# daovietanh190499/3D_Reconstruction

Measured on AMD Instinct MI355X. Metric: image-pairs matched/sec, higher is better.
Workload: dtype f32 descriptors: int8 MFMA certified filter + f64 re-score; 1 GPU; C3/C4 all-pairs BF-L2 + ratio 0.75: 257 imgs x 4096 kpts x 256-d, exact f32-input semantics (oracle.match.bf_match_exact, bit for bit); pairs=32896, api=dist.match_all_pairs_sharded(exact=True), match_mode=exact-float, parallelism=pairs/1

## Files before the change

### 3d_reconstruction_amd/csrc/fp6_sched.h

```cpp
#pragma once

namespace sfmhip {

template <int KK, int NS>
struct Fp6Sched {
    static constexpr int MPT = KK * NS;
    static constexpr int F = (KK - 1) * NS + 5;
    static constexpr int kBudget = KK == 1 ? 3 : 2;
    static_assert(F + 1 < MPT, "a spilled maximum reads its chain before the next tile rewrites it");
    static constexpr int chain(int g, int which) { return (g - F - which + MPT) % MPT; }
    static constexpr bool back(int g, int which) { return g - F - which < 0; }
    static constexpr int load(int g) { return (chain(g, 0) < NS) + (chain(g, 1) < NS); }
    static constexpr int before(int g, int which) {
        const int f = F + which, wrap = f + NS - MPT;
        return (g < wrap ? g : wrap) + (g > f ? g - f : 0);
    }
    static constexpr int merge(int h, int j) {
        const int g = h % MPT;
        const int k = (h / MPT) * (kBudget * MPT - 2 * NS) + kBudget * g - before(g, 0) - before(g, 1);
        return (j < kBudget - load(g) && k + j < 4 * NS) ? k + j : -1;
    }
    static constexpr int merge_chain(int k) { return 2 * (k / 8) + ((0xCA >> (k % 8)) & 1); }
    static constexpr int merge_step(int k) { return (0x3232'1100 >> (4 * (k % 8))) & 15; }
    static constexpr int kOwedFirst = MPT - F, kOwedSecond = MPT - F - 1;
    static constexpr bool merge_ready() {
        for (int c = 0; c < NS; ++c) {
            int h = 0;
            while (true) {
                bool found = false;
                for (int j = 0; j < kBudget; ++j) found |= merge(h, j) == 8 * (c / 2) + c % 2;
                if (found) break;
                ++h;
            }
            if (h < F + 1 + c - MPT) return false;
        }
        return true;
    }
};

__device__ __forceinline__ void fp6_merge_step(int step, float m, int rid, bool& up, float& w1, float& w2, int& wr) {
    const float a = w1, b = w2;
    const int r = wr;
    const bool u = up;
    if (step == 0) up = m > a;
    else if (step == 1) w2 = __builtin_amdgcn_fmed3f(a, b, m);
    else if (step == 2) wr = u ? rid : r;
    else w1 = u ? m : a;
}

}
```

### 3d_reconstruction_amd/csrc/match_dev.h

```cpp
#pragma once

#include "common.h"
#include <climits>

namespace sfmhip {

typedef int i32x2 __attribute__((ext_vector_type(2)));
typedef int i32x4 __attribute__((ext_vector_type(4)));
typedef int i32x8 __attribute__((ext_vector_type(8)));
typedef float f32x4 __attribute__((ext_vector_type(4)));

constexpr int kJB = 128;

template <int D>
__device__ __forceinline__ int swz_off(int r, int c) {
    constexpr int CPR = D / 16;
    constexpr int RPB = 256 / D;
    return r * D + ((c ^ ((r / RPB) % CPR)) << 4);
}

__device__ __forceinline__ int max3i(int a, int b, int c) {
    int r;
    asm("v_max3_i32 %0, %1, %2, %3" : "=v"(r) : "v"(a), "v"(b), "v"(c));
    return r;
}
__device__ __forceinline__ int med3i(int a, int b, int c) {
    int r;
    asm("v_med3_i32 %0, %1, %2, %3" : "=v"(r) : "v"(a), "v"(b), "v"(c));
    return r;
}

template <int D, int WAVES>
struct Stager {
    static constexpr int CPR = D / 16;
    static constexpr int RPB = 256 / D;
    static constexpr int TILE = kJB * D;
    static constexpr int NI = TILE / 1024;
    static constexpr int PER_WAVE = NI / WAVES;
    static constexpr int LDT = TILE / 16 / (64 * WAVES);
    static_assert(NI % WAVES == 0 && LDT >= 1, "block / workgroup mismatch");

    __device__ static void dma(const int8_t* src, const int32_t* ksrc, int8_t* dst, int32_t* kdst, int wave,
                               int lane) {
#pragma unroll
        for (int u = 0; u < PER_WAVE; ++u) {
            const int ins = wave * PER_WAVE + u;
            const int rows_per_ins = 1024 / D;
            const int r0 = ins * rows_per_ins;
            const int r = r0 + lane / CPR;
            const int c = (lane % CPR) ^ ((r / RPB) % CPR);
            __builtin_amdgcn_global_load_lds(
                (__attribute__((address_space(1))) void*)(src + (size_t)r * D + c * 16),
                (__attribute__((address_space(3))) void*)(dst + r0 * D), 16, 0, 0);
        }
        if (wave == WAVES - 1) {
#pragma unroll
            for (int u = 0; u < 2; ++u)
                __builtin_amdgcn_global_load_lds(
                    (__attribute__((address_space(1))) void*)(ksrc + u * 64 + lane),
                    (__attribute__((address_space(3))) void*)(kdst + u * 64), 4, 0, 0);
        }
    }
};

template <int MF> struct Mfma;
template <> struct Mfma<16> {
    using acc_t = i32x4;
    static constexpr int NREG = 4, KB = 64;
    __device__ static acc_t run(i32x4 a, i32x4 b, acc_t c) {
        return __builtin_amdgcn_mfma_i32_16x16x64_i8(a, b, c, 0, 0, 0);
    }
    __device__ static int row(int q, int grp) { return 4 * grp + q; }
};

struct CertArgs {
    const double* erow;
    const double* eimg;
    double inv_s;
    int force;
};
constexpr int kUndecidedBase = -3;
constexpr int kValueOnlyTiles = 4;
__device__ __forceinline__ int sqrt8_ceil(int d2) {
    const long long t = 64LL * d2;
    int u = (int)ceil(sqrt((double)t));
    while (u > 0 && (long long)(u - 1) * (u - 1) >= t) --u;
    while ((long long)u * u < t) ++u;
    return u;
}
template <typename OutT>
__device__ __forceinline__ int undecided_mark(int d2) {
    if constexpr (sizeof(OutT) == 2) return kUndecidedBase - sqrt8_ceil(d2);
    else return kUndecidedBase - d2;
}
template <typename OutT>
__device__ __forceinline__ double mark_sqrt_d2(int mark) {
    if constexpr (sizeof(OutT) == 2) return (double)(kUndecidedBase - mark) * 0.125;
    else return sqrt((double)(kUndecidedBase - mark));
}

__device__ __forceinline__ int certify(int d1lo, int d1hi, int d2lo, int d2hi, double E, double inv_s, double rn2,
                                       double rd2) {
    const double up = 1.0 + 0x1p-50, dn = 1.0 - 0x1p-50;
    const double s1l = sqrt((double)d1lo) * inv_s, s1h = sqrt((double)d1hi) * inv_s;
    const double s2l = sqrt((double)d2lo) * inv_s, s2h = sqrt((double)d2hi) * inv_s;
    const double a1 = fmax(s1l * dn - E * up, 0.0), b1 = (s1h + E) * up;
    const double a2 = fmax(s2l * dn - E * up, 0.0), b2 = (s2h + E) * up;
    const double wl = 1.0 - 1e-12, wh = 1.0 + 1e-12;
    const double lo1 = a1 * a1 * wl, hi1 = b1 * b1 * wh, lo2 = a2 * a2 * wl, hi2 = b2 * b2 * wh;
    if (rd2 * lo1 >= rn2 * hi2) return 0;
    if (hi1 < lo2 && rd2 * hi1 < rn2 * lo2) return 1;
    return -1;
}

template <int D, int MF, int NS, int VG, typename OutT>
__device__ __forceinline__ void value_only_tail(const int (&w1)[NS], const int (&w2)[NS], const int (&wr)[NS],
                                                const int8_t* __restrict__ desc, const int8_t* __restrict__ bdesc,
                                                const int32_t* __restrict__ bkeys, const int32_t* __restrict__ norms,
                                                int a, int b, int m_pad, int na_rows, int ibase, int grp, int lr,
                                                int lane, long long rn2, long long rd2, OutT* __restrict__ out_m,
                                                const CertArgs& ca) {
    constexpr int NG = 64 / MF;
    int v1 = INT_MIN, v2 = INT_MIN, loc = 0;
#pragma unroll
    for (int s = 0; s < NS; ++s) {
        int a1 = w1[s], a2 = w2[s], al = wr[s] * NG + grp;
#pragma unroll
        for (int off = MF; off < 64; off <<= 1) {
            const int o1 = __shfl_xor(a1, off), o2 = __shfl_xor(a2, off), ol = __shfl_xor(al, off);
            const bool mine = a1 > o1 || (a1 == o1 && al < ol);
            a2 = max3i(min(a1, o1), a2, o2);
            al = mine ? al : ol;
            a1 = max(a1, o1);
        }
        if (s == grp) { v1 = a1; v2 = a2; loc = al; }
    }
    const int i = ibase + grp * MF + lr;
    int res = -1, na = 0, du1 = 0, hidx = -1;
    double E = 0.0;
    bool survivor = false;
    if (i < na_rows) {
        na = norms[(size_t)a * m_pad + i];
        du1 = na - 2 * v1;
        const int du2ub = na - 2 * v2;
        E = ca.erow[(size_t)a * m_pad + i] + ca.eimg[b];
        if (ca.force)
            res = undecided_mark<OutT>(min(du2ub, D * 255 * 255));
        else
            survivor = certify(max(du1 - 1, 0), du1, max(du1 - 1, 0), du2ub, E, ca.inv_s, (double)rn2,
                               (double)rd2) != 0;
    }
    constexpr int NC = 4 * VG;
    constexpr int LPC = (64 / NC) < (D / 16) ? (64 / NC) : (D / 16);
    constexpr int BPL = D / LPC;
    const int c = min(lane / LPC, NC - 1), part = lane % LPC;
    unsigned long long bal = __ballot(survivor);
    while (bal) {
        const int l = __builtin_ctzll(bal);
        bal &= bal - 1;
        const int ri = __shfl(i, l), rv = __shfl(v1, l), rl = __shfl(loc, l);
        const int j0 = (rl / NG) * VG * MF + 4 * (rl % NG);
        const int j = j0 + (c >> 2) * MF + (c & 3);
        const int8_t* pa = desc + ((size_t)a * m_pad + ri) * D + part * BPL;
        const int8_t* pb = bdesc + (size_t)j * D + part * BPL;
        int dot = 0;
#pragma unroll
        for (int w = 0; w < BPL / 16; ++w) {
            const i32x4 x = *reinterpret_cast<const i32x4*>(pa + 16 * w);
            const i32x4 y = *reinterpret_cast<const i32x4*>(pb + 16 * w);
#pragma unroll
            for (int e = 0; e < 4; ++e) dot = __builtin_amdgcn_sdot4(x[e], y[e], dot, false);
        }
#pragma unroll
        for (int off = 1; off < LPC; off <<= 1) dot += __shfl_xor(dot, off);
        const int u = dot + bkeys[j];
        const bool hit = lane < NC * LPC && part == 0 && u == rv;
        const unsigned long long hb = __ballot(hit);
        int x = u == rv ? INT_MIN : u;
#pragma unroll
        for (int off = LPC; off < 64; off <<= 1) x = max(x, __shfl_xor(x, off));
        if (lane == l) {
            const bool one = __popcll(hb) == 1;
            v2 = max(v2, one ? x : rv);
            if (one) {
                const int hc = __builtin_ctzll(hb) / LPC;
                hidx = j0 + (hc >> 2) * MF + (hc & 3);
            }
        }
    }
    if (survivor) {
        const int du2 = na - 2 * v2;
        const int v = certify(max(du1 - 1, 0), du1, max(du2 - 1, 0), du2, E, ca.inv_s, (double)rn2, (double)rd2);
        res = v == 0 ? -1 : (v > 0 && hidx >= 0) ? hidx : undecided_mark<OutT>(du2);
    }
    if (i < m_pad) out_m[i] = (OutT)res;
}

constexpr int kMatchRows = 256;
constexpr int kMatchFp6Rows = 512;

struct FilterLaunch {
    const int8_t* desc;
    const int32_t* norms;
    const int32_t* keys;
    const int32_t* n_kpts;
    int m_pad, d;
    const int32_t* pairs;
    int n_iblk, nwg;
    long long rn2, rd2;
    CertArgs ca;
    hipStream_t stream;
    int32_t *dist1, *dist2;
    const uint8_t* dense;
    const float* hf;
};
template <typename OutT> int launch_match_cert(const FilterLaunch& f, OutT* matches0);
template <typename OutT> int launch_match_fp6(const FilterLaunch& f, OutT* matches0);
struct ResolveLaunch;
template <typename OutT> int launch_resolve(const ResolveLaunch& r, OutT* matches0);
void launch_key_values(const int32_t* keys, int64_t n, int32_t* h, float* hf, hipStream_t stream);

template <typename OutT>
inline int check_match_call(const char* entry, bool exact, int n_img, int P, int m_pad, int mode, int ratio_num,
                            int ratio_den, bool pointers, int rows_per_wg, int* n_iblk, int* nwg) {
    *n_iblk = *nwg = 0;
    SFMHIP_REQUIRE(n_img > 0 && P >= 0, "%s: bad counts", entry);
    SFMHIP_REQUIRE(m_pad > 0 && m_pad % kJB == 0, "%s: m_pad must be a positive multiple of 128", entry);
    if (exact) SFMHIP_REQUIRE(mode == 0 || mode == 1, "%s: mode must be 0 or 1", entry);
    SFMHIP_REQUIRE(ratio_num > 0 && ratio_den > 0 && ratio_num <= 65535 && ratio_den <= 65535,
                   "%s: ratio must be a positive fraction", entry);
    if constexpr (sizeof(OutT) == 2)
        SFMHIP_REQUIRE(m_pad <= 32767, "%s_i16: m_pad must be <= 32767 for an int16 graph", entry);
    if (P == 0) return SFMHIP_OK;
    SFMHIP_REQUIRE(pointers, "%s: null pointer", entry);
    *n_iblk = ceil_div(m_pad, rows_per_wg);
    const int64_t nwg64 = (int64_t)P * *n_iblk;
    SFMHIP_REQUIRE(nwg64 < INT_MAX, "%s: too many pairs for one launch", entry);
    *nwg = (int)nwg64;
    return SFMHIP_OK;
}

}
```

### 3d_reconstruction_amd/csrc/match_fp6.hip

```cpp
#include "match_dev.h"
#include "fp6_sched.h"

namespace sfmhip {

__device__ __forceinline__ int fp6_grid_index(float y, int* g) {
    const float t = fminf(fabsf(y), 60.f);
    int n, m;
    if (t < 16.f) { m = (int)__builtin_rintf(t); n = m; }
    else if (t < 32.f) { const int r = (int)__builtin_rintf(0.5f * t); m = 2 * r; n = r + 8; }
    else { const int r = (int)__builtin_rintf(0.25f * t); m = 4 * r; n = r + 16; }
    const bool neg = y < 0.f && m > 0;
    *g = neg ? -m : m;
    return n | (neg ? 32 : 0);
}
__global__ void quantize_fp6_kernel(const float* __restrict__ in, int64_t n_chunks, int d, int m_pad,
                                    const int32_t* __restrict__ nk, int8_t* __restrict__ g,
                                    uint8_t* __restrict__ code) {
    for (int64_t c = (int64_t)blockIdx.x * blockDim.x + threadIdx.x; c < n_chunks;
         c += (int64_t)gridDim.x * blockDim.x) {
        const int64_t e0 = c * 32, row = e0 / d;
        const int img = (int)(row / m_pad), r = (int)(row % m_pad);
        const bool valid = r < nk[img];
        unsigned gw[8], cw[8];
#pragma unroll
        for (int w = 0; w < 8; ++w) gw[w] = cw[w] = 0u;
        if (valid) {
#pragma unroll
            for (int q = 0; q < 8; ++q) {
                const float4 x = *reinterpret_cast<const float4*>(in + e0 + 4 * q);
                const float v[4] = {x.x, x.y, x.z, x.w};
                unsigned pk = 0u;
#pragma unroll
                for (int t = 0; t < 4; ++t) {
                    int gv;
                    const int cd = fp6_grid_index(127.f * v[t], &gv);
                    gw[q] |= (unsigned)(gv & 0xff) << (8 * t);
                    pk |= (unsigned)cd << (6 * t);
                }
#pragma unroll
                for (int t = 0; t < 3; ++t) {
                    const int byte = 3 * q + t;
                    cw[byte >> 2] |= ((pk >> (8 * t)) & 0xffu) << (8 * (byte & 3));
                }
            }
        }
        uint4* go = reinterpret_cast<uint4*>(g + e0);
        uint4* co = reinterpret_cast<uint4*>(code + e0);
        go[0] = make_uint4(gw[0], gw[1], gw[2], gw[3]);
        go[1] = make_uint4(gw[4], gw[5], gw[6], gw[7]);
        co[0] = make_uint4(cw[0], cw[1], cw[2], cw[3]);
        co[1] = make_uint4(cw[4], cw[5], cw[6], cw[7]);
    }
}


__global__ void pack_fp6_kernel(const uint8_t* __restrict__ code, int64_t n_chunks, int d,
                                uint8_t* __restrict__ dense) {
    const int spr = d / 32;
    for (int64_t c = (int64_t)blockIdx.x * blockDim.x + threadIdx.x; c < n_chunks;
         c += (int64_t)gridDim.x * blockDim.x) {
        const int64_t row = c / spr;
        const int s = (int)(c % spr);
        const uint4 lo = *reinterpret_cast<const uint4*>(code + c * 32);
        const uint2 hi = *reinterpret_cast<const uint2*>(code + c * 32 + 16);
        uint8_t* rp = dense + row * (3 * d / 4);
        *reinterpret_cast<uint4*>(rp + 16 * s) = lo;
        *reinterpret_cast<uint2*>(rp + d / 2 + 8 * s) = hi;
    }
}

template <int D, int WAVES>
struct DenseStager {
    static constexpr int ROW = 3 * D / 4, LB = D / 2, HB = D / 4;
    static constexpr int LO = kJB * LB, TILE = kJB * ROW;
    static constexpr int CPR = LB / 16, RPB = 256 / LB;
    static constexpr int UPR = HB / 16, RPH = 256 / HB;
    static constexpr int NLO = LO / 1024 / WAVES, NHI = (TILE - LO) / 1024 / WAVES;
    static_assert(NLO * WAVES * 1024 == LO && NHI * WAVES * 1024 == TILE - LO && NLO >= 1 && NHI >= 1,
                  "block / workgroup mismatch");
    static_assert(RPB * CPR == 16 && RPH * UPR == 16, "a 16-row tile covers every bank once");

    __device__ static int lo_sw(int r) { return ((((r & 15) + 4) >> 3) & 1) ^ ((r / RPB) % CPR); }
    __device__ static int hi_sw(int r) { return (r / RPH) % UPR; }
    __device__ static int lo_off(int r, int s) { return r * LB + ((s ^ lo_sw(r)) << 4); }
    __device__ static int hi_off(int r, int s) { return LO + r * HB + ((((s >> 1) ^ hi_sw(r)) << 4) | ((s & 1) << 3)); }

    struct Lanes {
        unsigned lo[NLO], hi[NHI], key;
    };
    __device__ static Lanes lanes(int wave, int lane) {
        Lanes l;
#pragma unroll
        for (int u = 0; u < NLO; ++u) {
            const int r = (wave * NLO + u) * (1024 / LB) + lane / CPR;
            l.lo[u] = (unsigned)(r * ROW + (((lane % CPR) ^ lo_sw(r)) << 4));
        }
#pragma unroll
        for (int u = 0; u < NHI; ++u) {
            const int r = (wave * NHI + u) * (1024 / HB) + lane / UPR;
            l.hi[u] = (unsigned)(r * ROW + LB + (((lane % UPR) ^ hi_sw(r)) << 4));
        }
        l.key = (unsigned)(lane * 4);
        return l;
    }

    __device__ static void dma(const uint8_t* src, const int32_t* ksrc, int8_t* dst, int32_t* kdst, int wave,
                               const Lanes& l) {
#pragma unroll
        for (int u = 0; u < NLO; ++u) {
            unsigned o = l.lo[u];
            asm volatile("" : "+v"(o));
            __builtin_amdgcn_global_load_lds((__attribute__((address_space(1))) void*)(src + o),
                                             (__attribute__((address_space(3))) void*)(dst + (wave * NLO + u) * 1024),
                                             16, 0, 0);
        }
#pragma unroll
        for (int u = 0; u < NHI; ++u) {
            unsigned o = l.hi[u];
            asm volatile("" : "+v"(o));
            __builtin_amdgcn_global_load_lds(
                (__attribute__((address_space(1))) void*)(src + o),
                (__attribute__((address_space(3))) void*)(dst + LO + (wave * NHI + u) * 1024), 16, 0, 0);
        }
        if (wave == WAVES - 1) {
#pragma unroll
            for (int u = 0; u < 2; ++u)
                __builtin_amdgcn_global_load_lds(
                    (__attribute__((address_space(1))) void*)(reinterpret_cast<const uint8_t*>(ksrc + u * 64) + l.key),
                    (__attribute__((address_space(3))) void*)(kdst + u * 64), 4, 0, 0);
        }
    }
};

__device__ __forceinline__ i32x2 lds_read_b64(const int8_t* p) {
    return *(const volatile __attribute__((address_space(3))) i32x2*)p;
}

struct Fp6Operand {
    i32x4 lo;
    i32x2 hi;
    __device__ i32x8 tuple() const { return i32x8{lo[0], lo[1], lo[2], lo[3], hi[0], hi[1], 0, 0}; }
};

constexpr int kFp6Tiles = 8;
constexpr int kFp6Waves = 4;

template <int D, typename OutT>
__global__ __launch_bounds__(64 * kFp6Waves, 2) void match_fp6_kernel(
    const uint8_t* __restrict__ dense, const int8_t* __restrict__ g, const int32_t* __restrict__ norms,
    const int32_t* __restrict__ h, const float* __restrict__ hf, const int32_t* __restrict__ nk, int m_pad,
    const int32_t* __restrict__ pairs, int n_iblk, int nwg, long long rn2, long long rd2,
    OutT* __restrict__ m0, CertArgs ca) {
    constexpr int MF = 16, NS = kFp6Tiles, WAVES = kFp6Waves, VG = kValueOnlyTiles;
    static_assert(D % 128 == 0, "one MFMA takes 128 elements of k");
    static_assert(NS % 4 == 0, "value_only_tail takes four query tiles at a time");
    using S = DenseStager<D, WAVES>;
    constexpr int KK = D / 128;
    using SC = Fp6Sched<KK, NS>;
    static_assert(kJB / MF == 2 * VG, "two ranges per block: the range maxima alternate between two sets");
    static_assert(SC::merge(VG * SC::MPT, 0) == -1, "a range's gaps hold the previous range's merge");
    static_assert(SC::merge_ready(), "a chain's merge starts behind its last maximum");
    constexpr int TILE = S::TILE;
    constexpr int NT = 64 * WAVES;
    constexpr int IW = MF * NS, IB = IW * WAVES;
    constexpr int JT = kJB / MF;
    constexpr int kScale = 0;
    constexpr float kLow = -262144.f;

    __shared__ __attribute__((aligned(16))) int8_t lds[2 * TILE + 2 * kJB * 4];

    const int wg = xcd_remap(blockIdx.x, nwg);
    const int pair = wg / n_iblk, ib = wg % n_iblk;
    const int a = pairs[2 * pair], b = pairs[2 * pair + 1];
    const int na_rows = nk[a], nb_rows = nk[b];
    const int tid = threadIdx.x, lane = tid & 63;
    const int wave = __builtin_amdgcn_readfirstlane(tid >> 6);
    const int grp = lane / MF, lr = lane % MF;
    const int ibase = ib * IB + wave * IW;
    OutT* out_m = m0 + (size_t)pair * m_pad;

    if (ib * IB >= na_rows || nb_rows < 2) {
        const int iend = min(ib * IB + IB, m_pad);
        for (int i = ib * IB + tid; i < iend; i += NT) out_m[i] = -1;
        return;
    }

    const uint8_t* bdense = dense + (size_t)b * m_pad * S::ROW;
    const int32_t* bhf = reinterpret_cast<const int32_t*>(hf) + (size_t)b * m_pad;
    const int nblk = (nb_rows + kJB - 1) / kJB;
    int32_t* kbase = reinterpret_cast<int32_t*>(lds + 2 * TILE);

    const typename S::Lanes dl = S::lanes(wave, lane);
    S::dma(bdense, bhf, lds, kbase, wave, dl);

    Fp6Operand bq[NS][KK];
#pragma unroll
    for (int s = 0; s < NS; ++s) {
        const int i = min(ibase + s * MF + lr, m_pad - 1);
        const uint8_t* rp = dense + ((size_t)a * m_pad + i) * S::ROW;
#pragma unroll
        for (int kk = 0; kk < KK; ++kk) {
            bq[s][kk].lo = *reinterpret_cast<const i32x4*>(rp + 16 * (kk * 4 + grp));
            bq[s][kk].hi = *reinterpret_cast<const i32x2*>(rp + S::LB + 8 * (kk * 4 + grp));
        }
    }
    int lo_b[KK], hi_b[KK];
#pragma unroll
    for (int kk = 0; kk < KK; ++kk) {
        lo_b[kk] = S::lo_off(lr, kk * 4 + grp);
        hi_b[kk] = S::hi_off(lr, kk * 4 + grp);
    }

    float w1[NS], w2[NS];
    int wr[NS];
    f32x4 acc[NS];
    float half[NS], rm[2][NS];
    bool up[NS];
    int rid_owed = 0;
#pragma unroll
    for (int s = 0; s < NS; ++s) {
        w1[s] = kLow; w2[s] = kLow; wr[s] = 0;
        acc[s] = f32x4{kLow, kLow, kLow, kLow};
        half[s] = rm[0][s] = rm[1][s] = kLow;
        up[s] = false;
    }
    auto merge_step = [&](int c, int step, float m, int rid) {
        fp6_merge_step(step, m, rid, up[c], w1[c], w2[c], wr[c]);
    };

    __syncthreads();

    const uint8_t* bsrc = bdense;
    const int32_t* ksrc = bhf;
    for (int blk = 0; blk < nblk; ++blk) {
        const int cur = blk & 1;
        bsrc += TILE;
        ksrc += kJB;
        if (blk + 1 < nblk)
            S::dma(bsrc, ksrc, lds + (cur ^ 1) * TILE, kbase + (cur ^ 1) * kJB, wave, dl);
        const int8_t* tl = lds + cur * TILE;
        const float* kl = reinterpret_cast<const float*>(kbase + cur * kJB);
        Fp6Operand av;
        av.lo = *reinterpret_cast<const i32x4*>(tl + lo_b[0]);
        av.hi = lds_read_b64(tl + hi_b[0]);
        f32x4 hv = *reinterpret_cast<const f32x4*>(kl + 4 * grp);
#pragma unroll
        for (int jt = 0; jt < JT; ++jt) {
            const int R = jt / VG, tt = jt % VG;
            f32x4 hv_n = hv;
#pragma unroll
            for (int kk = 0; kk < KK; ++kk) {
                Fp6Operand av_n = av;
                __builtin_amdgcn_sched_barrier(0);
#pragma unroll
                for (int s = 0; s < NS; ++s) {
                    acc[s] = __builtin_amdgcn_mfma_scale_f32_16x16x128_f8f6f4(av.tuple(), bq[s][kk].tuple(),
                                                                              kk == 0 ? hv : acc[s], 2, 2, 0, kScale, 0,
                                                                              kScale);
                    __builtin_amdgcn_sched_barrier(0);
                    if (s == 0) {
                        if (kk + 1 < KK) {
                            av_n.lo = *reinterpret_cast<const i32x4*>(tl + lo_b[kk + 1] + jt * MF * S::LB);
                            av_n.hi = lds_read_b64(tl + hi_b[kk + 1] + jt * MF * S::HB);
                        } else if (jt + 1 < JT) {
                            av_n.lo = *reinterpret_cast<const i32x4*>(tl + lo_b[0] + (jt + 1) * MF * S::LB);
                            av_n.hi = lds_read_b64(tl + hi_b[0] + (jt + 1) * MF * S::HB);
                            hv_n = *reinterpret_cast<const f32x4*>(kl + (jt + 1) * MF + 4 * grp);
                        }
                        __builtin_amdgcn_sched_barrier(0);
                    }
                    const int gp = kk * NS + s;
                    if (const int c = SC::chain(gp, 0); c < NS) {
                        const int of = tt - SC::back(gp, 0);
                        const float from = of < 0 ? rm[R ^ 1][c] : of == 0 ? kLow : rm[R][c];
                        half[c] = __builtin_fmaxf(__builtin_fmaxf(from, acc[c][0]), acc[c][1]);
                    }
                    if (const int c = SC::chain(gp, 1); c < NS)
                        rm[tt == 0 && SC::back(gp, 1) ? R ^ 1 : R][c] =
                            __builtin_fmaxf(__builtin_fmaxf(half[c], acc[c][2]), acc[c][3]);
#pragma unroll
                    for (int j = 0; j < SC::kBudget; ++j)
                        if (const int k = SC::merge(tt * SC::MPT + gp, j); k >= 0) {
                            __builtin_amdgcn_sched_barrier(0);
                            merge_step(SC::merge_chain(k), SC::merge_step(k), rm[R ^ 1][SC::merge_chain(k)], rid_owed);
                        }
                    __builtin_amdgcn_sched_barrier(0);
                }
                av = av_n;
            }
            hv = hv_n;
            if (tt == VG - 1) rid_owed = blk * (JT / VG) + R;
        }
        __syncthreads();
    }
#pragma unroll
    for (int s = SC::kOwedFirst; s < NS; ++s)
        half[s] = __builtin_fmaxf(__builtin_fmaxf(rm[1][s], acc[s][0]), acc[s][1]);
#pragma unroll
    for (int s = SC::kOwedSecond; s < NS; ++s)
        rm[1][s] = __builtin_fmaxf(__builtin_fmaxf(half[s], acc[s][2]), acc[s][3]);
#pragma unroll
    for (int s = 0; s < NS; ++s)
#pragma unroll
        for (int step = 0; step < 4; ++step) merge_step(s, step, rm[1][s], rid_owed);

#pragma unroll
    for (int q = 0; q < NS / 4; ++q) {
        int v1[4], v2[4], vr[4];
#pragma unroll
        for (int s = 0; s < 4; ++s) {
            v1[s] = (int)(64.f * w1[4 * q + s]);
            v2[s] = (int)(64.f * w2[4 * q + s]);
            vr[s] = wr[4 * q + s];
        }
        value_only_tail<D, MF, 4, VG, OutT>(v1, v2, vr, g, g + (size_t)b * m_pad * D, h + (size_t)b * m_pad, norms, a, b,
                                            m_pad, na_rows, ibase + q * 4 * MF, grp, lr, lane, rn2, rd2, out_m, ca);
    }
}

template <typename OutT>
int launch_match_fp6(const FilterLaunch& f, OutT* matches0) {
    static_assert(kMatchFp6Rows == 16 * kFp6Tiles * kFp6Waves, "query rows per workgroup");
    auto launch = [&](auto kern) {
        hipLaunchKernelGGL(kern, dim3(f.nwg), dim3(64 * kFp6Waves), 0, f.stream, f.dense, f.desc, f.norms, f.keys, f.hf,
                           f.n_kpts, f.m_pad, f.pairs, f.n_iblk, f.nwg, f.rn2, f.rd2, matches0, f.ca);
    };
    switch (f.d) {
        case 128: launch(match_fp6_kernel<128, OutT>); break;
        case 256: launch(match_fp6_kernel<256, OutT>); break;
        default: return SFMHIP_E_UNSUPPORTED;
    }
    return check_launch("match_kernel<cert>");
}
template int launch_match_fp6<int32_t>(const FilterLaunch&, int32_t*);
template int launch_match_fp6<int16_t>(const FilterLaunch&, int16_t*);

}

using namespace sfmhip;

extern "C" int sfmhip_desc_quantize_fp6(const float* in, int n_img, int m_pad, int d, const int32_t* n_kpts,
                                        int8_t* g, uint8_t* code, void* stream) {
    SFMHIP_REQUIRE(in && g && code && n_kpts, "sfmhip_desc_quantize_fp6: null pointer");
    SFMHIP_REQUIRE(n_img > 0 && m_pad > 0 && d > 0 && d % 32 == 0, "sfmhip_desc_quantize_fp6: bad shape");
    const int64_t n_chunks = (int64_t)n_img * m_pad * d / 32;
    const int grid = (int)std::min<int64_t>((n_chunks + 255) / 256, 4096);
    hipLaunchKernelGGL(quantize_fp6_kernel, dim3(grid), dim3(256), 0, as_stream(stream), in, n_chunks, d, m_pad,
                       n_kpts, g, code);
    return check_launch("quantize_fp6_kernel");
}

extern "C" int sfmhip_desc_pack_fp6(const uint8_t* code, int n_img, int m_pad, int d, uint8_t* dense, void* stream) {
    SFMHIP_REQUIRE(code && dense, "sfmhip_desc_pack_fp6: null pointer");
    SFMHIP_REQUIRE(n_img > 0 && m_pad > 0 && d > 0 && d % 64 == 0, "sfmhip_desc_pack_fp6: bad shape");
    const int64_t n_chunks = (int64_t)n_img * m_pad * d / 32;
    const int grid = (int)std::min<int64_t>((n_chunks + 255) / 256, 4096);
    hipLaunchKernelGGL(pack_fp6_kernel, dim3(grid), dim3(256), 0, as_stream(stream), code, n_chunks, d, dense);
    return check_launch("pack_fp6_kernel");
}
```

Baseline: 665,100 pairs/s.

## Make fp6 value-range width a per-D template parameter spanning blocks

The range width VG (column tiles per tracked maximum) becomes a template parameter chosen per descriptor size: four tiles for 256-d (unchanged from the former constant) and sixteen for 128-d, where a range now spans two blocks. The block loop is restructured into phase-specialised unrolled bodies so range sets alternate correctly across blocks, and the tail's re-scan is bounded by the last valid column. Wider ranges mean fewer merge steps in the main loop but more candidates to re-score per survivor in the tail. For the 256-d workload the default path keeps the same range size, so mainly the code structure changes.

```diff
diff --git a/3d_reconstruction_amd/csrc/fp6_sched.h b/3d_reconstruction_amd/csrc/fp6_sched.h
--- a/3d_reconstruction_amd/csrc/fp6_sched.h
+++ b/3d_reconstruction_amd/csrc/fp6_sched.h
@@ -36,6 +36,34 @@
         }
         return true;
     }
+    static constexpr bool merge_once(int tiles) {
+        int next = 0;
+        for (int h = 0; h < tiles * MPT; ++h) {
+            int n = load(h % MPT);
+            for (int j = 0; j < kBudget; ++j)
+                if (const int k = merge(h, j); k >= 0) {
+                    if (k != next) return false;
+                    ++next;
+                    ++n;
+                }
+            if (n > kBudget) return false;
+        }
+        return next == 4 * NS;
+    }
+};
+
+template <int VG, int JT>
+struct Fp6Range {
+    static_assert(VG >= 1 && (VG & (VG - 1)) == 0 && JT >= 1 && (JT & (JT - 1)) == 0, "powers of two");
+    static constexpr int PER = 2 * VG > JT ? 2 * VG / JT : 1;
+    static constexpr int set(int ph, int jt) { return ((ph * JT + jt) / VG) & 1; }
+    static constexpr int tile(int ph, int jt) { return (ph * JT + jt) % VG; }
+    static constexpr bool valid() {
+        if ((PER * JT) % (2 * VG) != 0 || set(PER - 1, JT - 1) != 1 || tile(PER - 1, JT - 1) != VG - 1) return false;
+        for (int ph = 0; ph < PER; ++ph)
+            if (tile(ph, JT - 1) == 0) return false;
+        return true;
+    }
 };
 
 __device__ __forceinline__ void fp6_merge_step(int step, float m, int rid, bool& up, float& w1, float& w2, int& wr) {
diff --git a/3d_reconstruction_amd/csrc/match_dev.h b/3d_reconstruction_amd/csrc/match_dev.h
--- a/3d_reconstruction_amd/csrc/match_dev.h
+++ b/3d_reconstruction_amd/csrc/match_dev.h
@@ -119,7 +119,7 @@
                                                 const int32_t* __restrict__ bkeys, const int32_t* __restrict__ norms,
                                                 int a, int b, int m_pad, int na_rows, int ibase, int grp, int lr,
                                                 int lane, long long rn2, long long rd2, OutT* __restrict__ out_m,
-                                                const CertArgs& ca) {
+                                                const CertArgs& ca, int j_end = INT_MAX) {
     constexpr int NG = 64 / MF;
     int v1 = INT_MIN, v2 = INT_MIN, loc = 0;
 #pragma unroll
@@ -160,7 +160,12 @@
         bal &= bal - 1;
         const int ri = __shfl(i, l), rv = __shfl(v1, l), rl = __shfl(loc, l);
         const int j0 = (rl / NG) * VG * MF + 4 * (rl % NG);
-        const int j = j0 + (c >> 2) * MF + (c & 3);
+        int j = j0 + (c >> 2) * MF + (c & 3);
+        bool seen = true;
+        if constexpr (VG * MF > kJB) {
+            seen = j < j_end;
+            j = seen ? j : j0;
+        }
         const int8_t* pa = desc + ((size_t)a * m_pad + ri) * D + part * BPL;
         const int8_t* pb = bdesc + (size_t)j * D + part * BPL;
         int dot = 0;
@@ -173,7 +178,7 @@
         }
 #pragma unroll
         for (int off = 1; off < LPC; off <<= 1) dot += __shfl_xor(dot, off);
-        const int u = dot + bkeys[j];
+        const int u = seen ? dot + bkeys[j] : INT_MIN;
         const bool hit = lane < NC * LPC && part == 0 && u == rv;
         const unsigned long long hb = __ballot(hit);
         int x = u == rv ? INT_MIN : u;
diff --git a/3d_reconstruction_amd/csrc/match_fp6.hip b/3d_reconstruction_amd/csrc/match_fp6.hip
--- a/3d_reconstruction_amd/csrc/match_fp6.hip
+++ b/3d_reconstruction_amd/csrc/match_fp6.hip
@@ -144,21 +144,46 @@
 
 constexpr int kFp6Tiles = 8;
 constexpr int kFp6Waves = 4;
-
-template <int D, typename OutT>
+#ifndef SFMHIP_FP6_RANGE_256
+#define SFMHIP_FP6_RANGE_256 4
+#endif
+#ifndef SFMHIP_FP6_RANGE_128
+#define SFMHIP_FP6_RANGE_128 16
+#endif
+template <int D>
+constexpr int kFp6RangeTiles = D == 256 ? SFMHIP_FP6_RANGE_256 : SFMHIP_FP6_RANGE_128;
+
+template <typename T>
+__device__ __forceinline__ void fp6_hold(T& x) {
+    asm volatile("" : "+v"(x));
+}
+
+template <typename T>
+__device__ __forceinline__ void fp6_hold_uniform(T& x) {
+    asm volatile("" : "+s"(x));
+}
+
+template <int K>
+struct Fp6Phase {
+    static constexpr int value = K;
+};
+
+template <int D, typename OutT, int VG = kFp6RangeTiles<D>>
 __global__ __launch_bounds__(64 * kFp6Waves, 2) void match_fp6_kernel(
     const uint8_t* __restrict__ dense, const int8_t* __restrict__ g, const int32_t* __restrict__ norms,
     const int32_t* __restrict__ h, const float* __restrict__ hf, const int32_t* __restrict__ nk, int m_pad,
     const int32_t* __restrict__ pairs, int n_iblk, int nwg, long long rn2, long long rd2,
     OutT* __restrict__ m0, CertArgs ca) {
-    constexpr int MF = 16, NS = kFp6Tiles, WAVES = kFp6Waves, VG = kValueOnlyTiles;
+    constexpr int MF = 16, NS = kFp6Tiles, WAVES = kFp6Waves;
     static_assert(D % 128 == 0, "one MFMA takes 128 elements of k");
     static_assert(NS % 4 == 0, "value_only_tail takes four query tiles at a time");
     using S = DenseStager<D, WAVES>;
     constexpr int KK = D / 128;
     using SC = Fp6Sched<KK, NS>;
-    static_assert(kJB / MF == 2 * VG, "two ranges per block: the range maxima alternate between two sets");
-    static_assert(SC::merge(VG * SC::MPT, 0) == -1, "a range's gaps hold the previous range's merge");
+    using RG = Fp6Range<VG, kJB / MF>;
+    static_assert(VG == 4 || VG == 8 || VG == 16, "ranges of half a block, one block or two blocks");
+    static_assert(RG::valid(), "the range maxima alternate between two sets by the parity of the range");
+    static_assert(SC::merge_once(VG < kJB / MF ? VG : kJB / MF), "a range's first gaps hold the previous range's merge, once");
     static_assert(SC::merge_ready(), "a chain's merge starts behind its last maximum");
     constexpr int TILE = S::TILE;
     constexpr int NT = 64 * WAVES;
@@ -230,23 +255,15 @@
 
     __syncthreads();
 
-    const uint8_t* bsrc = bdense;
-    const int32_t* ksrc = bhf;
-    for (int blk = 0; blk < nblk; ++blk) {
-        const int cur = blk & 1;
-        bsrc += TILE;
-        ksrc += kJB;
-        if (blk + 1 < nblk)
-            S::dma(bsrc, ksrc, lds + (cur ^ 1) * TILE, kbase + (cur ^ 1) * kJB, wave, dl);
-        const int8_t* tl = lds + cur * TILE;
-        const float* kl = reinterpret_cast<const float*>(kbase + cur * kJB);
+    auto block = [&](auto phase, int blk, const int8_t* tl, const float* kl) __attribute__((always_inline)) {
+        constexpr int PH = decltype(phase)::value;
         Fp6Operand av;
         av.lo = *reinterpret_cast<const i32x4*>(tl + lo_b[0]);
         av.hi = lds_read_b64(tl + hi_b[0]);
         f32x4 hv = *reinterpret_cast<const f32x4*>(kl + 4 * grp);
 #pragma unroll
         for (int jt = 0; jt < JT; ++jt) {
-            const int R = jt / VG, tt = jt % VG;
+            const int R = RG::set(PH, jt), tt = RG::tile(PH, jt);
             f32x4 hv_n = hv;
 #pragma unroll
             for (int kk = 0; kk < KK; ++kk) {
@@ -289,20 +306,81 @@
                 av = av_n;
             }
             hv = hv_n;
-            if (tt == VG - 1) rid_owed = blk * (JT / VG) + R;
-        }
+            if (tt == VG - 1) {
+                if constexpr (VG <= JT) rid_owed = blk * (JT / VG) + jt / VG;
+                else rid_owed = blk / (VG / JT);
+            }
+        }
+        if constexpr (RG::PER > 1) {
+#pragma unroll
+            for (int s = 0; s < NS; ++s) {
+                fp6_hold(acc[s]);
+                fp6_hold(half[s]); fp6_hold(rm[0][s]); fp6_hold(rm[1][s]);
+                fp6_hold(w1[s]); fp6_hold(w2[s]); fp6_hold(wr[s]);
+            }
+        }
+    };
+
+    const uint8_t* bsrc = bdense;
+    const int32_t* ksrc = bhf;
+    auto step = [&](auto phase, int blk) __attribute__((always_inline)) {
+        const int cur = blk & 1;
+        bsrc += TILE;
+        ksrc += kJB;
+        if constexpr (RG::PER > 1) {
+            fp6_hold_uniform(bsrc);
+            fp6_hold_uniform(ksrc);
+        }
+        if (blk + 1 < nblk)
+            S::dma(bsrc, ksrc, lds + (cur ^ 1) * TILE, kbase + (cur ^ 1) * kJB, wave, dl);
+        block(phase, blk, lds + cur * TILE, reinterpret_cast<const float*>(kbase + cur * kJB));
         __syncthreads();
+    };
+    if constexpr (RG::PER == 1) {
+        for (int blk = 0; blk < nblk; ++blk) step(Fp6Phase<0>{}, blk);
+    } else if constexpr (RG::PER == 2) {
+        int blk = 0;
+        for (; blk + 2 <= nblk; blk += 2) {
+            step(Fp6Phase<0>{}, blk);
+            step(Fp6Phase<1>{}, blk + 1);
+        }
+        if (blk < nblk) step(Fp6Phase<0>{}, blk);
+    } else {
+        static_assert(RG::PER == 4, "one body per phase");
+        int blk = 0;
+        for (; blk + 4 <= nblk; blk += 4) {
+            step(Fp6Phase<0>{}, blk);
+            step(Fp6Phase<1>{}, blk + 1);
+            step(Fp6Phase<2>{}, blk + 2);
+            step(Fp6Phase<3>{}, blk + 3);
+        }
+        if (blk < nblk) {
+            step(Fp6Phase<0>{}, blk);
+            if (blk + 1 < nblk) {
+                step(Fp6Phase<1>{}, blk + 1);
+                if (blk + 2 < nblk) step(Fp6Phase<2>{}, blk + 2);
+            }
+        }
+    }
+    const int last_tile = nblk * JT - 1;
+    const bool set1 = VG < JT || ((last_tile / VG) & 1);
+    if constexpr (VG > JT) rid_owed = last_tile / VG;
+    float rl[NS];
+#pragma unroll
+    for (int s = 0; s < NS; ++s) {
+        const float r0 = rm[0][s], r1 = rm[1][s];
+        rl[s] = set1 ? r1 : r0;
     }
 #pragma unroll
     for (int s = SC::kOwedFirst; s < NS; ++s)
-        half[s] = __builtin_fmaxf(__builtin_fmaxf(rm[1][s], acc[s][0]), acc[s][1]);
+        half[s] = __builtin_fmaxf(__builtin_fmaxf(rl[s], acc[s][0]), acc[s][1]);
 #pragma unroll
     for (int s = SC::kOwedSecond; s < NS; ++s)
-        rm[1][s] = __builtin_fmaxf(__builtin_fmaxf(half[s], acc[s][2]), acc[s][3]);
+        rl[s] = __builtin_fmaxf(__builtin_fmaxf(half[s], acc[s][2]), acc[s][3]);
 #pragma unroll
     for (int s = 0; s < NS; ++s)
 #pragma unroll
-        for (int step = 0; step < 4; ++step) merge_step(s, step, rm[1][s], rid_owed);
+        for (int step = 0; step < 4; ++step) merge_step(s, step, rl[s], rid_owed);
 
 #pragma unroll
     for (int q = 0; q < NS / 4; ++q) {
@@ -314,7 +392,8 @@
             vr[s] = wr[4 * q + s];
         }
         value_only_tail<D, MF, 4, VG, OutT>(v1, v2, vr, g, g + (size_t)b * m_pad * D, h + (size_t)b * m_pad, norms, a, b,
-                                            m_pad, na_rows, ibase + q * 4 * MF, grp, lr, lane, rn2, rd2, out_m, ca);
+                                            m_pad, na_rows, ibase + q * 4 * MF, grp, lr, lane, rn2, rd2, out_m, ca,
+                                            nblk * kJB);
     }
 }
 
```

Result: no change. 664,200 pairs/s (-0.1%).
